# rvolden/C3POa

Measured on AMD Instinct MI355X. Metric: R2C2 reads->consensus/sec, higher is better.
Workload: dtype int32

## Files before the change

### c3poa_amd/csrc/c3_args.h

```cpp
#pragma once
#include "c3_dev.h"
#include <cstddef>

struct C3Counters {
  int queue;
  int peaks_queue;
  unsigned long long cells;
  unsigned long long cells_computed;
  unsigned long long zero_cells;
  int poa_ovf;
  int poa_ovf16;
  int n_windows;
  int win_ovf;
  int win_queue2;
  int band_layers, band_fallback;
  int band_mismatch;
  struct { int window, layer, R, q, band_row, full_row, next_row; } verify;
  unsigned long long phases[16];
};
static_assert(offsetof(C3Counters, cells) % 8 == 0 && offsetof(C3Counters, cells_computed) % 8 == 0 &&
              offsetof(C3Counters, zero_cells) % 8 == 0 && offsetof(C3Counters, phases) % 8 == 0, "u64 counters must be 8-byte aligned");

struct ConkArgs {
  C3Batch b; const uint8_t* sp_codes; const int* sp_len; int32_t* track; C3Info* info; C3Counters* cnt;
  int match, mismatch, penalty;
  int n_spl; int32_t* scan;
};
struct PeaksArgs {
  C3Batch b; const int32_t* track; C3Info* info; double* bufA; double* bufB; int32_t* cand; uint8_t* cstate;
  int32_t* raw_peaks; int32_t* n_raw; const int* sp_len; double coef[64]; int64_t maxL; int window, iters, min_dist;
  C3Counters* cnt;
};
struct PoaArgs {
  C3Batch b; C3Info* info; C3Params p; C3Counters* cnt; const int* work; int n_work;
  int* ibase; int* ebase; char* cellsb; uint8_t* bbase; long long* score;
  int Ncap, K, Pcap, cells_cap;
  uint8_t* draft; int32_t* tpos; uint8_t* msa_dbg; const int64_t* msa_off; int* msa_len;
  int rb_span;
  int no2col;
  uint4* desc; int* jump;
  int* pbase;
  int* overflow;
  int* overflow16;
};
#define C3_POA_NI 19
__host__ __device__ inline int c3_poa_far_shift(bool w32) { return w32 ? 0 : 2; }
struct PoaLayout { size_t ints, edges, cells, bases, score, desc, jump, path, total; };
__host__ __device__ inline PoaLayout c3_poa_layout(size_t Ncap, size_t K, int cells_cap, int far_shift, size_t Pcap) {
  PoaLayout l;
  l.ints = sizeof(int) * C3_POA_NI * Ncap; l.edges = sizeof(int) * 3 * Ncap * K;
  l.cells = 2 * (size_t)cells_cap + 16 * (size_t)(cells_cap >> far_shift);
  l.bases = 5 * Ncap; l.score = sizeof(long long) * Ncap; l.desc = sizeof(uint4) * 2 * Ncap;
  l.jump = sizeof(int) * C3_JUMP_LEVELS * Ncap; l.path = sizeof(int) * Pcap;
  l.total = l.ints + l.edges + l.cells + l.bases + l.score + l.desc + l.jump + l.path;
  return l;
}

struct WLayer { int qbeg, len, begin, end; };
struct WinRec { int rid, w, n_layers, blen, tgs, out_len, polished, pad_; };
struct PrepArgs {
  C3Batch b; C3Info* info; C3Params p; C3Counters* cnt; const int* work; int n_work;
  const uint8_t* draft; int32_t* tpos; int wcap; uint8_t* eD; int64_t ecap; int* lw_first; int* lw_last; int NLcap, NWcap;
  WinRec* wrec; WLayer* wlay; int* win_base;
  int sub_shift;
  int rows_old;
};
struct WinArgs {
  C3Batch b; C3Params p; C3Counters* cnt; int n_win; const WinRec* wrec_in; WinRec* wrec; const WLayer* wlay; int NLcap;
  const uint8_t* draft;
  uint8_t* base; int* ibase; int* ebase; long long* score;
  int32_t* H; uint16_t* D; uint4* rdesc; int Ncap, K; long long hcap; uint8_t* wout; int wout_cap;
  int Lcap;
  int band_mode;
  const int* wlist; int* ovf_list;
  int no_chain;
};
#define W_INTS 19
struct WinLayout { size_t ints, edges, bases, score, H, D, desc, total; };
__host__ __device__ inline WinLayout c3_win_layout(size_t Ncap, size_t K, size_t hcap) {
  WinLayout l;
  l.ints = sizeof(int) * W_INTS * Ncap; l.edges = sizeof(int) * 4 * Ncap * K; l.bases = 2 * Ncap; l.score = sizeof(long long) * Ncap;
  l.H = sizeof(int32_t) * hcap; l.D = hcap; l.desc = sizeof(uint4) * (Ncap + 1);
  l.total = l.ints + l.edges + l.bases + l.score + l.H + l.D + l.desc;
  return l;
}
struct StitchArgs {
  C3Batch b; C3Info* info; const int* work; int n_work; const WinRec* wrec; const int* win_base; const uint8_t* wout; int wout_cap; char* cons;
  const uint8_t* zflag;
};
struct AdapterArgs {
  C3Batch b; C3Params p; C3Counters* cnt;
  const uint8_t* ad_codes; const int* ad_len; int n_ad;
  uint8_t* D; long long dcap;
  int32_t* out;
};

struct ZeroArgs {
  C3Batch b; C3Info* info; C3Params p; C3Counters* cnt; const int* work; int n_work;
  uint8_t* D; long long dcap;
  int4* zinfo; uint8_t* zflag;
  const uint8_t* draft; char* cons;
  uint8_t* S; long long scap; int zk;
};

struct ZlLayout { long long ck, dir, car, total; };
__host__ __device__ inline ZlLayout c3_zl_layout(long long n0, long long n1, long long K) {
  ZlLayout l;
  l.ck = 0;
  l.dir = (n1 + K - 1) / K * (n0 + 1) * 8;
  l.car = (l.dir + (n1 < K ? n1 : K) * (n0 + 1) + 15) & ~15LL;
  l.total = (l.car + n1 * 12 + 255) & ~255LL;
  return l;
}
struct QvArgs {
  int n_reads; const C3Info* info; const uint32_t* pk; const int64_t* woff; const uint8_t* qual; const int64_t* off;
  const char* cons; char* qv;
  int sa_np, sa_n; const int64_t* sa_woff; const int64_t* sa_off; const int32_t* sa_mode;
  uint32_t* dirs; long long dir_words;
  int* gS; uint8_t* gcodes; long long gcap;
  int lds_n;
  unsigned long long* cnt;
};
```

### c3poa_amd/csrc/c3_stages.hip

```cpp
#include "c3_host.h"

__global__ void k_summary(const C3Info* info, const int64_t* off, int n, Summary* out) {
  int i = blockIdx.x * blockDim.x + threadIdx.x;
  if (i >= n) return;
  const C3Info* p = &info[i];
  Summary s; s.status = p->status; s.n_sub = p->n_sub; s.max_sub = 0; s.sum_sub = 0; s.max_dang = 0; s.n_peaks = p->n_peaks;
  for (int k = 0; k < p->n_sub; ++k) { int l = p->sub_end[k] - p->sub_beg[k]; s.sum_sub += l; if (l > s.max_sub) s.max_sub = l; }
  int L = (int)(off[i + 1] - off[i]);
  s.front = p->has_front ? p->front_end : 0; s.tail = p->has_tail ? L - p->tail_beg : 0;
  if (p->has_front) s.max_dang = p->front_end;
  if (p->has_tail && L - p->tail_beg > s.max_dang) s.max_dang = L - p->tail_beg;
  out[i] = s;
}

static hipError_t zero_counters(c3_handle* h) { return hipMemsetAsync(h->d_counter.p, 0, sizeof(C3Counters), h->stream); }

static int auto_slots(c3_handle* h, int want, size_t per_slot_bytes, int n_items, int waves_per_cu) {
  int s = want > 0 ? want : h->n_cus * waves_per_cu;
  size_t budget = h->mem_total ? h->mem_total / 3 : ((size_t)64 << 30);
  if (per_slot_bytes > 0) { size_t mx = budget / per_slot_bytes; if ((size_t)s > mx) s = (int)std::max<size_t>(mx, 1); }
  if (s > n_items) s = std::max(n_items, 1);
  return s;
}

static int run_conk(c3_handle* h) {
  HIPCHK(h->d_track.ensure(sizeof(int32_t) * (size_t)h->total + 64));
  HIPCHK(zero_cnt(h, &dev_cnt(h)->queue));
  ConkArgs a; a.b = dev_batch(h); a.sp_codes = h->d_sp_codes.as<uint8_t>(); a.sp_len = h->d_sp_len.as<int>();
  a.track = h->d_track.as<int32_t>(); a.info = h->d_info.as<C3Info>(); a.cnt = dev_cnt(h);
  a.match = h->cfg.conk_match; a.mismatch = h->cfg.conk_mismatch; a.penalty = h->cfg.conk_penalty; a.n_spl = h->n_spl; a.scan = nullptr;
  int waves = std::min(h->n, h->n_cus * 32);
  c3k_launch_conk(&a, h->max_spl, (waves + 3) / 4, 0, h->stream);
  HIPCHK(hipGetLastError());
  return 0;
}

static void savgol_coeffs(int window, double* c) {
  int m = (window - 1) / 2;
  double den = (double)(2 * m - 1) * (double)(2 * m + 1) * (double)(2 * m + 3);
  for (int k = -m; k <= 0; ++k) c[k + m] = 3.0 * (double)(3 * m * m + 3 * m - 1 - 5 * k * k) / den;
}

static int run_peaks(c3_handle* h) {
  static const int blocks_per_cu = c3k_peaks_blocks_per_cu();
  const int grid = std::min(h->n, h->n_cus * blocks_per_cu);
  h->peaks_grid = grid;
  const size_t mL = (size_t)h->maxL + 8;
  HIPCHK(h->d_bufA.ensure(sizeof(double) * mL * grid)); HIPCHK(h->d_bufB.ensure(sizeof(double) * mL * grid));
  HIPCHK(h->d_cand.ensure(sizeof(int32_t) * (mL / 2 + 2) * grid)); HIPCHK(h->d_cst.ensure((mL / 2 + 2) * grid));
  HIPCHK(h->d_raw.ensure(sizeof(int32_t) * (size_t)h->n * C3_MAX_PEAKS)); HIPCHK(h->d_nraw.ensure(sizeof(int32_t) * (size_t)h->n));
  PeaksArgs a; memset(&a, 0, sizeof(a));
  a.b = dev_batch(h); a.track = h->d_track.as<int32_t>(); a.info = h->d_info.as<C3Info>();
  a.bufA = h->d_bufA.as<double>(); a.bufB = h->d_bufB.as<double>(); a.cand = h->d_cand.as<int32_t>(); a.cstate = h->d_cst.as<uint8_t>();
  a.raw_peaks = h->d_raw.as<int32_t>(); a.n_raw = h->d_nraw.as<int32_t>(); a.sp_len = h->d_sp_len.as<int>();
  savgol_coeffs(h->cfg.sg_window, a.coef);
  a.maxL = (int64_t)mL; a.window = h->cfg.sg_window; a.iters = h->cfg.sg_iters; a.min_dist = h->cfg.mdistcutoff;
  a.cnt = dev_cnt(h);
  HIPCHK(zero_cnt(h, &a.cnt->peaks_queue));
  c3k_launch_peaks(&a, grid, h->stream);
  HIPCHK(hipGetLastError());
  return 0;
}

static int copy_summary(c3_handle* h) {
  const int n = h->n;
  HIPCHK(h->d_sum.ensure(sizeof(Summary) * (size_t)n));
  hipLaunchKernelGGL(k_summary, dim3((n + 255) / 256), dim3(256), 0, h->stream, h->d_info.as<C3Info>(), h->d_off.as<int64_t>(), n, h->d_sum.as<Summary>());
  h->sum.resize(n);
  HIPCHK(hipMemcpyAsync(h->sum.data(), h->d_sum.p, sizeof(Summary) * (size_t)n, hipMemcpyDeviceToHost, h->stream));
  if (!getenv("C3_NO_SPIN")) {
    hipError_t q;
    while ((q = hipStreamQuery(h->stream)) == hipErrorNotReady) { for (int k_ = 0; k_ < 64; ++k_) __builtin_ia32_pause(); }
    if (q != hipSuccess) HIPCHK(q);
  }
  HIPCHK(hipStreamSynchronize(h->stream));
  int k = 2;
  for (int i = 0; i < n; ++i) k = std::max(k, std::max(h->sum[i].n_peaks, h->sum[i].n_sub));
  h->res_prefix = std::min((k + 7) & ~7, (int)C3_MAX_PEAKS);
  return 0;
}

static void fill_zero_args(c3_handle* h, ZeroArgs& z, int nz) {
  memset(&z, 0, sizeof(z));
  z.b = dev_batch(h); z.info = h->d_info.as<C3Info>(); z.p = dev_params(h->cfg); z.cnt = dev_cnt(h);
  z.work = h->d_zwork.as<int>(); z.n_work = nz;
  z.D = h->s_zero_d.as<uint8_t>(); z.zinfo = h->d_zinfo.as<int4>(); z.zflag = h->d_zflag.as<uint8_t>();
  z.draft = h->d_draft.as<uint8_t>(); z.cons = h->d_cons.as<char>();
}

static const long long ZL_BUDGET = 1LL << 30;
static int run_zero(c3_handle* h) {
  h->zwork.clear();
  HIPCHK(h->d_zflag.ensure((size_t)h->n + 16));
  HIPCHK(hipMemsetAsync(h->d_zflag.p, 0, (size_t)h->n, h->stream));
  if (!h->cfg.zero || h->injected) return 0;
  const char* ev_long = getenv("C3_DEBUG_ZERO_LONG");
  const bool force_long = ev_long && atoi(ev_long) != 0;
  const char* ev_k = getenv("C3_DEBUG_ZERO_K");
  const int zk = (ev_k && atoi(ev_k) > 0) ? atoi(ev_k) : 256;
  long long dmax = 0, smax = 0;
  std::vector<int> zlong;
  for (int i = 0; i < h->n; ++i) {
    const Summary& s = h->sum[i];
    if (s.status != C3_ST_NO_CONSENSUS || s.n_sub != 0 || s.front <= 0 || s.tail <= 0) continue;
    const long long cells = (long long)s.front * s.tail;
    if (cells > h->cfg.zero_max_cells) continue;
    if (!force_long && s.front <= 4096 && cells <= (16 << 20)) {
      h->zwork.push_back(i);
      dmax = std::max(dmax, (long long)(s.front + 1) * (s.tail + 1));
    } else {
      zlong.push_back(i);
      smax = std::max(smax, c3_zl_layout(s.front, s.tail, zk).total);
    }
  }
  const int ns = (int)h->zwork.size(), nl = (int)zlong.size();
  h->zwork.insert(h->zwork.end(), zlong.begin(), zlong.end());
  const int nz = ns + nl;
  if (nz == 0) return 0;
  HIPCHK(h->d_zwork.ensure(sizeof(int) * (size_t)nz)); HIPCHK(h->d_zinfo.ensure(sizeof(int4) * (size_t)h->n));
  if (ns) {
    const int grid = std::min(ns, 512);
    HIPCHK(h->s_zero_d.ensure((size_t)dmax * grid + 64));
  }
  int grid_l = 0;
  if (nl) {
    grid_l = (int)std::min<long long>(std::min(nl, 2 * h->n_cus), std::max(1LL, ZL_BUDGET / smax));
    HIPCHK(h->s_zero_l.ensure((size_t)smax * grid_l));
  }
  HIPCHK(hipMemcpyAsync(h->d_zwork.p, h->zwork.data(), sizeof(int) * (size_t)nz, hipMemcpyHostToDevice, h->stream));
  if (ns) {
    ZeroArgs z; fill_zero_args(h, z, ns); z.dcap = dmax;
    DBG("zero: nz=%d grid=%d dmax=%lld\n", ns, std::min(ns, 512), dmax);
    c3k_launch_zero(&z, std::min(ns, 512), h->stream);
    HIPCHK(hipGetLastError());
  }
  if (nl) {
    ZeroArgs z; fill_zero_args(h, z, nl);
    z.work = h->d_zwork.as<int>() + ns; z.S = h->s_zero_l.as<uint8_t>(); z.scap = smax; z.zk = zk;
    DBG("zero long: nz=%d grid=%d slot=%lld K=%d\n", nl, grid_l, smax, zk);
    c3k_launch_zero_long(&z, grid_l, h->stream);
    HIPCHK(hipGetLastError());
  }
  { int r_ = copy_summary(h); DBG("zero done\n"); return r_; }
}

static int fetch_summary(c3_handle* h) {
  int rc = copy_summary(h);
  DBG("summary copied\n");
  if (rc) return rc;
  const auto wl0 = std::chrono::steady_clock::now();
  struct WlTimer { c3_handle* h; std::chrono::steady_clock::time_point t0; ~WlTimer() { h->tm.ms_host_worklist = std::chrono::duration<float, std::milli>(std::chrono::steady_clock::now() - t0).count(); } } wl_timer_{h, wl0};
  HIPCHK(zero_cnt(h, &dev_cnt(h)->zero_cells));
  if ((rc = run_zero(h))) return rc;
  const int n = h->n;
  h->work.clear();
  for (int i = 0; i < n; ++i) if (h->sum[i].status == C3_ST_OK && h->sum[i].n_sub >= 1) h->work.push_back(i);
  if (n < (1 << 24)) {
    const size_t m = h->work.size();
    std::vector<uint64_t> keys(m), tmp(m);
    for (size_t k = 0; k < m; ++k) {
      const int i = h->work[k];
      const uint64_t cost = (uint64_t)h->sum[i].sum_sub * (uint64_t)h->sum[i].n_sub;
      keys[k] = ((((uint64_t)1 << 40) - 1 - cost) << 24) | (uint64_t)i;
    }
    uint64_t* src = keys.data(); uint64_t* dst = tmp.data();
    for (int pass = 0; pass < 4; ++pass) {
      const int sh = 24 + 10 * pass;
      size_t cnt[1025] = {0};
      for (size_t k = 0; k < m; ++k) ++cnt[((src[k] >> sh) & 1023) + 1];
      for (int b = 0; b < 1024; ++b) cnt[b + 1] += cnt[b];
      for (size_t k = 0; k < m; ++k) dst[cnt[(src[k] >> sh) & 1023]++] = src[k];
      std::swap(src, dst);
    }
    for (size_t k = 0; k < m; ++k) h->work[k] = (int)(src[k] & 0xffffff);
  } else {
    std::stable_sort(h->work.begin(), h->work.end(), [&](int x, int y) {
      long cx = (long)h->sum[x].sum_sub * h->sum[x].n_sub, cy = (long)h->sum[y].sum_sub * h->sum[y].n_sub; return cx > cy; });
  }
  HIPCHK(h->d_work.ensure(sizeof(int) * std::max<size_t>(h->work.size(), 1)));
  if (!h->work.empty()) HIPCHK(hipMemcpyAsync(h->d_work.p, h->work.data(), sizeof(int) * h->work.size(), hipMemcpyHostToDevice, h->stream));
  return 0;
}

static int launch_poa(c3_handle* h, const int* d_work, int nw, int Ncap, int K, int Pcap, long long cells, int* d_overflow, int* d_overflow16, int waves_per_cu, int wide_ring) {
  cells = (cells + 15) & ~15LL;
  cells = (cells + 63) & ~63LL;
  const bool w32 = d_overflow16 == nullptr || getenv("C3_DEBUG_POA32");
  const PoaLayout L = c3_poa_layout(Ncap, K, (int)cells, c3_poa_far_shift(w32), Pcap);
  const int slots = auto_slots(h, h->cfg.slots_poa, L.total, nw, waves_per_cu);
  const size_t S = (size_t)slots;
  HIPCHK(h->s_poa_i.ensure(L.ints * S)); HIPCHK(h->s_poa_nk.ensure(L.edges * S));
  HIPCHK(h->s_poa_cells.ensure(L.cells * S + 256)); HIPCHK(h->s_poa_b.ensure(L.bases * S)); HIPCHK(h->s_poa_sc.ensure(L.score * S));
  HIPCHK(h->s_poa_desc.ensure(L.desc * S)); HIPCHK(h->s_poa_jump.ensure(L.jump * S)); HIPCHK(h->s_poa_path.ensure(L.path * S));
  PoaArgs a; memset(&a, 0, sizeof(a));
  a.b = dev_batch(h); a.info = h->d_info.as<C3Info>(); a.p = dev_params(h->cfg);
  a.cnt = dev_cnt(h); a.work = d_work; a.n_work = nw;
  a.ibase = h->s_poa_i.as<int>(); a.ebase = h->s_poa_nk.as<int>(); a.cellsb = h->s_poa_cells.as<char>();
  a.bbase = h->s_poa_b.as<uint8_t>(); a.score = h->s_poa_sc.as<long long>();
  a.Ncap = Ncap; a.K = K; a.Pcap = Pcap; a.cells_cap = (int)cells; a.desc = h->s_poa_desc.as<uint4>(); a.jump = h->s_poa_jump.as<int>();
  a.pbase = h->s_poa_path.as<int>(); a.overflow = d_overflow; a.overflow16 = d_overflow16;
  if (const char* e = getenv("C3_DEBUG_POA_RBSPAN")) a.rb_span = std::max(3300, atoi(e));
  a.no2col = getenv("C3_DEBUG_POA_NO2COL") != nullptr;
  a.draft = h->d_draft.as<uint8_t>(); a.tpos = h->d_tpos.as<int32_t>();
  a.msa_dbg = nullptr; a.msa_off = nullptr; a.msa_len = nullptr;
  if (h->debug_msa) { a.msa_dbg = h->d_msa.as<uint8_t>(); a.msa_off = h->d_msa_off.as<int64_t>(); a.msa_len = h->d_msa_len.as<int>(); }
  DBG("poa: nw=%d Ncap=%d K=%d cells=%lld slots=%d (%.1f MB per slot)%s\n", nw, Ncap, K, cells, slots, L.total / 1048576.0, d_overflow ? "" : (d_overflow16 ? " [full-size pass]" : " [32-bit pass]"));
  c3k_launch_poa(&a, slots, w32 ? 1 : 0, wide_ring, h->stream);
  HIPCHK(hipGetLastError());
  return 0;
}
// ... 268 lines not shown
```

### c3poa_amd/csrc/k_peaks.hip

```cpp
#include "c3_dev.h"
#include "c3_args.h"
#include "c3_launch.h"

#define PK_T 256
#define SG_T 1024
#define SG_H 64


__device__ __forceinline__ double sg_pad(const double* y, int n, int half, int x) {
  if (x < half) return y[0] - fabs(y[half - x] - y[0]);
  if (x >= n + half) return y[n - 1] + fabs(y[n - 2 - (x - n - half)] - y[n - 1]);
  return y[x - half];
}

__device__ __forceinline__ uint64_t dkey(double v) {
  uint64_t u = (uint64_t)__double_as_longlong(v);
  return (u >> 63) ? ~u : (u | 0x8000000000000000ull);
}
__device__ __forceinline__ double dunkey(uint64_t k) {
  uint64_t u = (k >> 63) ? (k & 0x7fffffffffffffffull) : ~k;
  return __longlong_as_double((long long)u);
}

__device__ __forceinline__ unsigned block_excl_scan(unsigned v, int* sh4, unsigned* total) {
  const int tid = threadIdx.x, lane = tid & 63, wv = tid >> 6;
  const unsigned inc = (unsigned)wave_scan_add((int)v);
  if (lane == 63) sh4[wv] = (int)inc;
  __syncthreads();
  unsigned base = 0, tot = 0;
#pragma unroll
  for (int w = 0; w < PK_T / 64; ++w) { const unsigned t = (unsigned)sh4[w]; if (w < wv) base += t; tot += t; }
  __syncthreads();
  *total = tot;
  return base + inc - v;
}

__device__ uint64_t block_select(const double* x, int n, int k, unsigned* hist, int* sh_i, uint64_t* keys ) {
  const int tid = threadIdx.x, lane = tid & 63;
  uint64_t prefix = 0, mask = 0;
  for (int pass = 7; pass >= 0; --pass) {
    const int shift = pass * 8;
    hist[tid] = 0;
    __syncthreads();
    for (int i0 = 0; i0 < n; i0 += 4 * PK_T) {
      double xv[4];
#pragma unroll
      for (int u = 0; u < 4; ++u) { const int i = i0 + u * PK_T + tid; xv[u] = i < n ? x[i] : 0.0; }
#pragma unroll
      for (int u = 0; u < 4; ++u) {
        const int i = i0 + u * PK_T + tid;
        const uint64_t key = dkey(xv[u]);
        const bool match = i < n && (key & mask) == prefix;
        const unsigned bin = (unsigned)(key >> shift) & 255u;
        unsigned long long todo = __ballot(match);
        for (int it = 0; it < 2 && todo; ++it) {
          const int l = __builtin_ctzll(todo);
          const unsigned b = (unsigned)__builtin_amdgcn_readlane((int)bin, l);
          const unsigned long long m = __ballot(match && bin == b) & todo;
          if (lane == l) atomicAdd(&hist[b], (unsigned)__popcll(m));
          todo &= ~m;
        }
        if (match && ((todo >> lane) & 1ull)) atomicAdd(&hist[bin], 1u);
      }
    }
    __syncthreads();
    {
      const unsigned c = hist[tid];
      unsigned tot;
      const unsigned cum = block_excl_scan(c, sh_i + 2, &tot);
      if (cum <= (unsigned)k && (unsigned)k < cum + c) { sh_i[0] = tid; sh_i[1] = (int)cum; sh_i[6] = (int)c; }
      if (tid == PK_T - 1 && (unsigned)k >= tot) { sh_i[0] = 255; sh_i[1] = (int)tot; sh_i[6] = INT32_MAX; }
    }
    __syncthreads();
    prefix |= (uint64_t)sh_i[0] << shift;
    mask |= (uint64_t)0xff << shift;
    k -= sh_i[1];
    const int cb = sh_i[6];
    __syncthreads();
    if (pass > 0 && cb <= PK_T) {
      if (tid == 0) sh_i[7] = 0;
      __syncthreads();
      for (int i0 = 0; i0 < n; i0 += 4 * PK_T) {
        double xv[4];
#pragma unroll
        for (int u = 0; u < 4; ++u) { const int i = i0 + u * PK_T + tid; xv[u] = i < n ? x[i] : 0.0; }
#pragma unroll
        for (int u = 0; u < 4; ++u) {
          const int i = i0 + u * PK_T + tid;
          const uint64_t key = dkey(xv[u]);
          if (i < n && (key & mask) == prefix) keys[atomicAdd(&sh_i[7], 1)] = key;
        }
      }
      __syncthreads();
      const uint64_t mine = tid < cb ? keys[tid] : ~0ull;
      int rank = 0;
      for (int j = 0; j < cb; ++j) { const uint64_t o = keys[j]; rank += (o < mine) || (o == mine && j < tid); }
      if (tid < cb && rank == k) *(uint64_t*)hist = mine;
      __syncthreads();
      const uint64_t r = *(const uint64_t*)hist;
      __syncthreads();
      return r;
    }
  }
  return prefix;
}

__device__ __forceinline__ int c3_rounding(int x, int base) {
  int q = x / base, r = x % base;
  if (2 * r < base) return q * base;
  if (2 * r > base) return (q + 1) * base;
  return ((q & 1) ? q + 1 : q) * base;
}

__global__ __launch_bounds__(PK_T) void k_peaks(PeaksArgs a) {
  __shared__ __attribute__((aligned(8))) unsigned hist[256];
  __shared__ int sh_i[8];
  __shared__ double sh_d[PK_T];
  __shared__ int sh_idx[PK_T];
  __shared__ int sh_cnt[PK_T + 1];
  __shared__ int kept[C3_MAX_PEAKS + 1];
  __shared__ double tb0[SG_T + 2 * SG_H], tb1[SG_T + 2 * SG_H];
  const int tid = threadIdx.x;
  double* A = a.bufA + (size_t)blockIdx.x * a.maxL;
  double* B = a.bufB + (size_t)blockIdx.x * a.maxL;
  int32_t* cand = a.cand + (size_t)blockIdx.x * (a.maxL / 2 + 2);
  uint8_t* cst = a.cstate + (size_t)blockIdx.x * (a.maxL / 2 + 2);
  const int half = (a.window - 1) / 2;

  __shared__ int s_rid;
  for (;;) {
    __syncthreads();
    if (tid == 0) s_rid = atomicAdd(&a.cnt->peaks_queue, 1);
    __syncthreads();
    const int rid = s_rid;
    if (rid >= a.b.n) break;
    C3Info* info = &a.info[rid];
    if (info->status == C3_ST_NOT_ASSIGNED) { if (tid == 0) a.n_raw[rid] = 0; continue; }
    const int64_t off = a.b.off[rid];
    const int n = (int)(a.b.off[rid + 1] - off);
    if (n < half + 1 || n < 2) { if (tid == 0) { info->status = C3_ST_TOO_SHORT; a.n_raw[rid] = 0; } continue; }
    const int32_t* tr = a.track + off;
    double* src = A; double* dst = B;
    const int H = a.iters * half;
    if (a.iters >= 1 && H <= SG_H) {
      double* xout = (a.iters & 1) ? B : A;
      for (int t0 = 0; t0 < n; t0 += SG_T) {
        const int base = t0 - H;
        const int T = min(SG_T, n - t0);
        for (int x = tid; x < T + 2 * H; x += PK_T) { const int g = base + x; if (g >= 0 && g < n) tb0[x] = (double)tr[g]; }
        __syncthreads();
        double* sb = tb0; double* db = tb1;
        for (int it = 0; it < a.iters; ++it) {
          const int ext = (a.iters - 1 - it) * half;
          const int glo = max(0, t0 - ext), ghi = min(n, t0 + T + ext);
          const bool last = it == a.iters - 1;
          const double* yv = sb - base;
          for (int g = glo + tid; g < ghi; g += PK_T) {
            double acc = 0.0;
            if (g >= half && g + half < n) {
              const double* y = yv + (g - half);
              if (half == 20) {
#pragma unroll
                for (int k = 0; k < 20; ++k) acc = __builtin_fma(a.coef[k], y[k] + y[40 - k], acc);
                acc = __builtin_fma(a.coef[20], y[20], acc);
              } else {
                for (int k = 0; k < half; ++k) acc = __builtin_fma(a.coef[k], y[k] + y[2 * half - k], acc);
                acc = __builtin_fma(a.coef[half], y[half], acc);
              }
            } else {
              for (int k = 0; k < half; ++k)
                acc = __builtin_fma(a.coef[k], sg_pad(yv, n, half, g + k) + sg_pad(yv, n, half, g + 2 * half - k), acc);
              acc = __builtin_fma(a.coef[half], sg_pad(yv, n, half, g + half), acc);
            }
            if (last) xout[g] = acc; else db[g - base] = acc;
          }
          __syncthreads();
          double* t = sb; sb = db; db = t;
        }
      }
      src = xout;
      __syncthreads();
    } else {
    for (int i = tid; i < n; i += PK_T) A[i] = (double)tr[i];
    __syncthreads();
    for (int it = 0; it < a.iters; ++it) {
      for (int i = tid; i < n; i += PK_T) {
        double acc = 0.0;
        if (i >= half && i + half < n) {
          const double* y = src + (i - half);
          for (int k = 0; k < half; ++k) acc = __builtin_fma(a.coef[k], y[k] + y[2 * half - k], acc);
          acc = __builtin_fma(a.coef[half], y[half], acc);
        } else {
          for (int k = 0; k < half; ++k)
            acc = __builtin_fma(a.coef[k], sg_pad(src, n, half, i + k) + sg_pad(src, n, half, i + 2 * half - k), acc);
          acc = __builtin_fma(a.coef[half], sg_pad(src, n, half, i + half), acc);
        }
        dst[i] = acc;
      }
      __syncthreads();
      double* t = src; src = dst; dst = t;
    }
    }
    const double* x = src;
    double med;
    {
#ifdef C3_EXP_X2_SEL
      { volatile uint64_t sink_ = block_select(x, n, (n - 1) / 3, hist, sh_i, (uint64_t*)sh_d); (void)sink_; }
#endif
      uint64_t k1 = block_select(x, n, (n - 1) / 2, hist, sh_i, (uint64_t*)sh_d);
      double v1 = dunkey(k1);
      if (n & 1) med = v1;
      else {
        int cnt_le = 0; uint64_t mn = ~0ull;
        for (int i = tid; i < n; i += PK_T) {
          uint64_t key = dkey(x[i]);
          if (key <= k1) ++cnt_le; else if (key < mn) mn = key;
        }
        sh_cnt[tid] = cnt_le; sh_d[tid] = __longlong_as_double((long long)mn);
        __syncthreads();
        for (int s = PK_T / 2; s > 0; s >>= 1) {
          if (tid < s) {
            sh_cnt[tid] += sh_cnt[tid + s];
            uint64_t o = (uint64_t)__double_as_longlong(sh_d[tid + s]), m = (uint64_t)__double_as_longlong(sh_d[tid]);
            if (o < m) sh_d[tid] = sh_d[tid + s];
          }
          __syncthreads();
        }
        int tot_le = sh_cnt[0]; uint64_t mnk = (uint64_t)__double_as_longlong(sh_d[0]);
        __syncthreads();
        double v2 = (tot_le > n / 2) ? v1 : dunkey(mnk);
        med = (v1 + v2) / 2.0;
      }
    }
    double mx = -1.0e308;
    for (int i = tid; i < n; i += PK_T) mx = fmax(mx, x[i]);
    sh_d[tid] = mx;
    __syncthreads();
    for (int s = PK_T / 2; s > 0; s >>= 1) { if (tid < s) sh_d[tid] = fmax(sh_d[tid], sh_d[tid + s]); __syncthreads(); }
    mx = sh_d[0];
    __syncthreads();
    int n_kept = 0;
    if (!(mx < 6 * med)) {
      const double height = med * 3;
      const int chunk = (n + PK_T - 1) / PK_T;
      const int lo = max(1, tid * chunk), hi = min(n - 1, (tid + 1) * chunk);
      int cnt = 0;
      for (int pass = 0; pass < 2; ++pass) {
        int w = (pass == 1) ? sh_cnt[tid] : 0;
        for (int i = lo; i < hi; ++i) {
          if (x[i - 1] < x[i]) {
            int ia = i + 1;
            while (ia < n - 1 && x[ia] == x[i]) ++ia;
            if (x[ia] < x[i] && x[i] >= height) {
              if (pass == 0) ++cnt; else { cand[w] = (i + ia - 1) / 2; cst[w] = 1; ++w; }
            }
          }
        }
        if (pass == 0) {
          unsigned tot;
          const unsigned ex = block_excl_scan((unsigned)cnt, sh_i + 2, &tot);
          sh_cnt[tid] = (int)ex;
          if (tid == 0) sh_cnt[PK_T] = (int)tot;
          __syncthreads();
        }
      }
      const int nc = sh_cnt[PK_T];
      __syncthreads();
      const int dist = a.min_dist < 1 ? 1 : a.min_dist;
      for (;;) {
        double bv = -1.0e308; int bi = -1;
        for (int c = tid; c < nc; c += PK_T)
          if (cst[c] == 1) { double v = x[cand[c]]; if (v > bv || (v == bv && c > bi)) { bv = v; bi = c; } }
        sh_d[tid] = bv; sh_idx[tid] = bi;
        __syncthreads();
        for (int s = PK_T / 2; s > 0; s >>= 1) {
          if (tid < s) {
            double ov = sh_d[tid + s]; int oi = sh_idx[tid + s];
            if (oi >= 0 && (sh_idx[tid] < 0 || ov > sh_d[tid] || (ov == sh_d[tid] && oi > sh_idx[tid]))) { sh_d[tid] = ov; sh_idx[tid] = oi; }
          }
          __syncthreads();
        }
        const int win = sh_idx[0];
        __syncthreads();
        if (win < 0) break;
        const int wp = cand[win];
        if (tid == 0) { cst[win] = 2; if (n_kept < C3_MAX_PEAKS) kept[n_kept] = wp; }
        ++n_kept;
        for (int c = tid; c < nc; c += PK_T)
          if (cst[c] == 1) { int dlt = cand[c] - wp; if (dlt < 0) dlt = -dlt; if (dlt < dist) cst[c] = 0; }
        __syncthreads();
      }
    }
    if (tid == 0) {
      int status = C3_ST_OK;
      if (n_kept > C3_MAX_PEAKS - 1) { status = C3_ST_LIMIT; n_kept = 0; }
      for (int i = 1; i < n_kept; ++i) { int v = kept[i], k = i - 1; while (k >= 0 && kept[k] > v) { kept[k + 1] = kept[k]; --k; } kept[k + 1] = v; }
      a.n_raw[rid] = n_kept;
      for (int i = 0; i < n_kept; ++i) a.raw_peaks[(size_t)rid * C3_MAX_PEAKS + i] = kept[i];
      const int S = a.sp_len[a.b.splint_id[rid]];
      int np = 0;
      for (int i = 0; i < n_kept; ++i) { int p = kept[i] + S / 2; if (p < n) info->peaks[np++] = p; }
      info->n_peaks = np;
      int ns = 0, hf = 0, ht = 0, fe = 0, tb = 0;
      if (status == C3_ST_OK && np == 0) status = C3_ST_NO_PEAKS;
      if (np > 1) {
        const int nl = np - 1;
        int* r = sh_idx;
        int* srt = sh_cnt;
        for (int i = 0; i < nl; ++i) srt[i] = r[i] = c3_rounding(info->peaks[i + 1] - info->peaks[i], 50);
        for (int i = 1; i < nl; ++i) { int v = srt[i], k = i - 1; while (k >= 0 && srt[k] > v) { srt[k + 1] = srt[k]; --k; } srt[k + 1] = v; }
        const double med2 = (nl & 1) ? (double)srt[nl / 2] : ((double)srt[nl / 2 - 1] + (double)srt[nl / 2]) / 2.0;
        const double lo8 = med2 * 0.8, hi12 = med2 * 1.2;
        for (int i = 0; i < nl; ++i)
          if (lo8 <= (double)r[i] && (double)r[i] <= hi12) { info->sub_beg[ns] = info->peaks[i]; info->sub_end[ns] = info->peaks[i + 1]; ++ns; }
        if (info->peaks[0] > 100) { hf = 1; fe = info->peaks[0]; }
        if (n - info->peaks[np - 1] > 100) { ht = 1; tb = info->peaks[np - 1]; }
      } else if (np == 1) {
        hf = 1; fe = info->peaks[0]; ht = 1; tb = info->peaks[0];
      }
      info->n_sub = ns; info->has_front = hf; info->has_tail = ht; info->front_end = fe; info->tail_beg = tb;
      if (status == C3_ST_OK && ns == 0) status = C3_ST_NO_CONSENSUS;
      if (status == C3_ST_OK && ns > C3_MAX_SUB) status = C3_ST_LIMIT;
      info->status = status;
    }
    __syncthreads();
  }
}

extern "C" int c3k_peaks_blocks_per_cu(void) {
  int nb = 0;
  if (hipOccupancyMaxActiveBlocksPerMultiprocessor(&nb, k_peaks, PK_T, 0) != hipSuccess || nb < 1) { (void)hipGetLastError(); nb = 4; }
  return nb;
}
extern "C" void c3k_launch_peaks(const PeaksArgs* a, int grid, hipStream_t stream) {
  hipLaunchKernelGGL(k_peaks, dim3(grid), dim3(PK_T), 0, stream, *a);
}
```

Before: 426,800.

## Use sample-bucket median and LDS candidate peak picking in peaks kernel

Replaces the eight-pass radix selection for the median with a sample-based bucket histogram that gathers only the median's bucket into shared memory, falling back to radix select when the bucket overflows. The max is now folded into the final FIR pass. Peak candidates are collected into shared memory and picked by a single wave, with no global cand/cstate passes or block-wide reductions, and the old path is kept as an overflow fallback. It also sets waves_per_eu, reuses the FIR tiles as scratch, and uses a per-read buffer row when the grid covers every read. This adds code complexity and fallback branches, and the changed shared-memory aliasing and tie-breaking could alter results.

```diff
diff --git a/c3poa_amd/csrc/c3_args.h b/c3poa_amd/csrc/c3_args.h
--- a/c3poa_amd/csrc/c3_args.h
+++ b/c3poa_amd/csrc/c3_args.h
@@ -30,7 +30,12 @@
   C3Batch b; const int32_t* track; C3Info* info; double* bufA; double* bufB; int32_t* cand; uint8_t* cstate;
   int32_t* raw_peaks; int32_t* n_raw; const int* sp_len; double coef[64]; int64_t maxL; int window, iters, min_dist;
   C3Counters* cnt;
+  int kcap;
+  int ccap;
+  int old_path;
 };
+#define C3_PEAKS_KCAP 1152
+#define C3_PEAKS_CCAP 1024
 struct PoaArgs {
   C3Batch b; C3Info* info; C3Params p; C3Counters* cnt; const int* work; int n_work;
   int* ibase; int* ebase; char* cellsb; uint8_t* bbase; long long* score;
diff --git a/c3poa_amd/csrc/c3_stages.hip b/c3poa_amd/csrc/c3_stages.hip
--- a/c3poa_amd/csrc/c3_stages.hip
+++ b/c3poa_amd/csrc/c3_stages.hip
@@ -43,7 +43,8 @@
 
 static int run_peaks(c3_handle* h) {
   static const int blocks_per_cu = c3k_peaks_blocks_per_cu();
-  const int grid = std::min(h->n, h->n_cus * blocks_per_cu);
+  int grid = std::min(h->n, h->n_cus * blocks_per_cu);
+  if (const char* g = getenv("C3_DEBUG_PEAKS_GRID")) grid = std::max(1, std::min(grid, atoi(g)));
   h->peaks_grid = grid;
   const size_t mL = (size_t)h->maxL + 8;
   HIPCHK(h->d_bufA.ensure(sizeof(double) * mL * grid)); HIPCHK(h->d_bufB.ensure(sizeof(double) * mL * grid));
@@ -56,6 +57,10 @@
   savgol_coeffs(h->cfg.sg_window, a.coef);
   a.maxL = (int64_t)mL; a.window = h->cfg.sg_window; a.iters = h->cfg.sg_iters; a.min_dist = h->cfg.mdistcutoff;
   a.cnt = dev_cnt(h);
+  const char* dbg = getenv("C3_DEBUG_PEAKS"); const char* kc = getenv("C3_DEBUG_PEAKS_KCAP"); const char* cc = getenv("C3_DEBUG_PEAKS_CCAP");
+  a.old_path = dbg && !strcmp(dbg, "old");
+  a.kcap = kc ? std::min(std::max(atoi(kc), 1), C3_PEAKS_KCAP) : C3_PEAKS_KCAP;
+  a.ccap = cc ? std::min(std::max(atoi(cc), 1), C3_PEAKS_CCAP) : C3_PEAKS_CCAP;
   HIPCHK(zero_cnt(h, &a.cnt->peaks_queue));
   c3k_launch_peaks(&a, grid, h->stream);
   HIPCHK(hipGetLastError());
diff --git a/c3poa_amd/csrc/k_peaks.hip b/c3poa_amd/csrc/k_peaks.hip
--- a/c3poa_amd/csrc/k_peaks.hip
+++ b/c3poa_amd/csrc/k_peaks.hip
@@ -5,6 +5,11 @@
 #define PK_T 256
 #define SG_T 1024
 #define SG_H 64
+#define PK_TB (SG_T + 2 * SG_H)
+#define PK_NB 1024
+static_assert(PK_NB == 4 * PK_T && PK_NB * sizeof(unsigned) <= PK_TB * sizeof(double), "one thread scans four buckets; histogram inside tile 0");
+static_assert(C3_PEAKS_KCAP <= PK_TB, "the gathered bucket aliases the second FIR tile");
+static_assert(C3_PEAKS_CCAP <= PK_TB && C3_PEAKS_CCAP * sizeof(int) <= PK_TB * sizeof(double), "candidate values alias tile 0, positions tile 1");
 
 
 __device__ __forceinline__ double sg_pad(const double* y, int n, int half, int x) {
@@ -22,8 +27,8 @@
   return __longlong_as_double((long long)u);
 }
 
-__device__ __forceinline__ unsigned block_excl_scan(unsigned v, int* sh4, unsigned* total) {
-  const int tid = threadIdx.x, lane = tid & 63, wv = tid >> 6;
+__device__ __forceinline__ unsigned block_excl_scan(int tid, unsigned v, int* sh4, unsigned* total) {
+  const int lane = tid & 63, wv = tid >> 6;
   const unsigned inc = (unsigned)wave_scan_add((int)v);
   if (lane == 63) sh4[wv] = (int)inc;
   __syncthreads();
@@ -35,8 +40,27 @@
   return base + inc - v;
 }
 
-__device__ uint64_t block_select(const double* x, int n, int k, unsigned* hist, int* sh_i, uint64_t* keys ) {
-  const int tid = threadIdx.x, lane = tid & 63;
+__device__ __forceinline__ void hist_add(int tid, unsigned* hist, bool match, unsigned bin) {
+  const int lane = tid & 63;
+  unsigned long long todo = __ballot(match);
+  for (int it = 0; it < 2 && todo; ++it) {
+    const int l = __builtin_ctzll(todo);
+    const unsigned b = (unsigned)__builtin_amdgcn_readlane((int)bin, l);
+    const unsigned long long m = __ballot(match && bin == b) & todo;
+    if (lane == l) atomicAdd(&hist[b], (unsigned)__popcll(m));
+    todo &= ~m;
+  }
+  if (match && ((todo >> lane) & 1ull)) atomicAdd(&hist[bin], 1u);
+}
+
+__device__ __forceinline__ void rank_two(int tid, const uint64_t mine, const uint64_t* keys, int cb, int ka, int kb, uint64_t* res) {
+  int rank = 0;
+  for (int j = 0; j < cb; ++j) { const uint64_t o = keys[j]; rank += (o < mine) || (o == mine && j < tid); }
+  if (tid < cb && rank == ka) res[0] = mine;
+  if (tid < cb && rank == kb) res[1] = mine;
+}
+
+__device__ uint64_t block_select(int tid, const double* x, int n, int k, unsigned* hist, int* sh_i, uint64_t* keys ) {
   uint64_t prefix = 0, mask = 0;
   for (int pass = 7; pass >= 0; --pass) {
     const int shift = pass * 8;
@@ -50,24 +74,14 @@
       for (int u = 0; u < 4; ++u) {
         const int i = i0 + u * PK_T + tid;
         const uint64_t key = dkey(xv[u]);
-        const bool match = i < n && (key & mask) == prefix;
-        const unsigned bin = (unsigned)(key >> shift) & 255u;
-        unsigned long long todo = __ballot(match);
-        for (int it = 0; it < 2 && todo; ++it) {
-          const int l = __builtin_ctzll(todo);
-          const unsigned b = (unsigned)__builtin_amdgcn_readlane((int)bin, l);
-          const unsigned long long m = __ballot(match && bin == b) & todo;
-          if (lane == l) atomicAdd(&hist[b], (unsigned)__popcll(m));
-          todo &= ~m;
-        }
-        if (match && ((todo >> lane) & 1ull)) atomicAdd(&hist[bin], 1u);
+        hist_add(tid, hist, i < n && (key & mask) == prefix, (unsigned)(key >> shift) & 255u);
       }
     }
     __syncthreads();
     {
       const unsigned c = hist[tid];
       unsigned tot;
-      const unsigned cum = block_excl_scan(c, sh_i + 2, &tot);
+      const unsigned cum = block_excl_scan(tid, c, sh_i + 2, &tot);
       if (cum <= (unsigned)k && (unsigned)k < cum + c) { sh_i[0] = tid; sh_i[1] = (int)cum; sh_i[6] = (int)c; }
       if (tid == PK_T - 1 && (unsigned)k >= tot) { sh_i[0] = 255; sh_i[1] = (int)tot; sh_i[6] = INT32_MAX; }
     }
@@ -92,10 +106,7 @@
         }
       }
       __syncthreads();
-      const uint64_t mine = tid < cb ? keys[tid] : ~0ull;
-      int rank = 0;
-      for (int j = 0; j < cb; ++j) { const uint64_t o = keys[j]; rank += (o < mine) || (o == mine && j < tid); }
-      if (tid < cb && rank == k) *(uint64_t*)hist = mine;
+      rank_two(tid, tid < cb ? keys[tid] : ~0ull, keys, cb, k, k + 1, (uint64_t*)hist);
       __syncthreads();
       const uint64_t r = *(const uint64_t*)hist;
       __syncthreads();
@@ -103,6 +114,137 @@
     }
   }
   return prefix;
+}
+
+__device__ double median_radix(int tid, const double* x, int n, unsigned* hist, int* sh_i, double* sh_d, int* sh_cnt) {
+#ifdef C3_EXP_X2_SEL
+  { volatile uint64_t sink_ = block_select(tid, x, n, (n - 1) / 3, hist, sh_i, (uint64_t*)sh_d); (void)sink_; }
+#endif
+  const uint64_t k1 = block_select(tid, x, n, (n - 1) / 2, hist, sh_i, (uint64_t*)sh_d);
+  const double v1 = dunkey(k1);
+  if (n & 1) return v1;
+  int cnt_le = 0; uint64_t mn = ~0ull;
+  for (int i = tid; i < n; i += PK_T) {
+    uint64_t key = dkey(x[i]);
+    if (key <= k1) ++cnt_le; else if (key < mn) mn = key;
+  }
+  sh_cnt[tid] = cnt_le; sh_d[tid] = __longlong_as_double((long long)mn);
+  __syncthreads();
+  for (int s = PK_T / 2; s > 0; s >>= 1) {
+    if (tid < s) {
+      sh_cnt[tid] += sh_cnt[tid + s];
+      uint64_t o = (uint64_t)__double_as_longlong(sh_d[tid + s]), m = (uint64_t)__double_as_longlong(sh_d[tid]);
+      if (o < m) sh_d[tid] = sh_d[tid + s];
+    }
+    __syncthreads();
+  }
+  const int tot_le = sh_cnt[0]; const uint64_t mnk = (uint64_t)__double_as_longlong(sh_d[0]);
+  __syncthreads();
+  const double v2 = (tot_le > n / 2) ? v1 : dunkey(mnk);
+  return (v1 + v2) / 2.0;
+}
+
+__device__ bool median_buckets(int tid, const double* x, int n, int kcap, double* med,
+                               unsigned* bh , double* vals , unsigned* hist, int* sh_i, double* sh_d) {
+  const int lane = tid & 63, wv = tid >> 6;
+  const int k = (n - 1) / 2;
+  const bool even = !(n & 1);
+  uint64_t* res = (uint64_t*)hist;
+  int B = 0, kk = k, cb = n;
+  double lo = 0.0, s = 0.0;
+#define PK_BUCKET(v) ({ const double t_ = ((v) - lo) * s; t_ >= (double)(PK_NB - 1) ? PK_NB - 1 : max((int)t_, 0); })
+  if (n > PK_T) {
+    uint64_t* skeys = (uint64_t*)sh_d;
+    const uint64_t mine = dkey(x[(int)(((long long)tid * n) >> 8)]);
+    skeys[tid] = mine;
+    __syncthreads();
+    rank_two(tid, mine, skeys, PK_T, PK_T / 4, 3 * PK_T / 4 - 1, res);
+    __syncthreads();
+    lo = dunkey(res[0]);
+    const double hi = dunkey(res[1]);
+    if (!(hi > lo)) { __syncthreads(); return false; }
+    s = (double)PK_NB / (hi - lo);
+    if (!(s < 1.0e300)) { __syncthreads(); return false; }
+#pragma unroll
+    for (int u = 0; u < 4; ++u) bh[u * PK_T + tid] = 0;
+    __syncthreads();
+    for (int i0 = 0; i0 < n; i0 += 4 * PK_T) {
+      double xv[4];
+#pragma unroll
+      for (int u = 0; u < 4; ++u) { const int i = i0 + u * PK_T + tid; xv[u] = i < n ? x[i] : lo; }
+#pragma unroll
+      for (int u = 0; u < 4; ++u) {
+        const bool in = i0 + u * PK_T + tid < n;
+        const int b = PK_BUCKET(xv[u]);
+        const unsigned long long m0 = __ballot(in && b == 0), m1 = __ballot(in && b == PK_NB - 1);
+        if (lane == 0 && m0) atomicAdd(&bh[0], (unsigned)__popcll(m0));
+        if (lane == 0 && m1) atomicAdd(&bh[PK_NB - 1], (unsigned)__popcll(m1));
+        if (in && b != 0 && b != PK_NB - 1) atomicAdd(&bh[b], 1u);
+      }
+    }
+    __syncthreads();
+    {
+      unsigned c[4], sum = 0, tot;
+#pragma unroll
+      for (int u = 0; u < 4; ++u) { c[u] = bh[4 * tid + u]; sum += c[u]; }
+      unsigned cum = block_excl_scan(tid, sum, sh_i + 2, &tot);
+#pragma unroll
+      for (int u = 0; u < 4; ++u) {
+        if (cum <= (unsigned)k && (unsigned)k < cum + c[u]) { sh_i[0] = 4 * tid + u; sh_i[1] = (int)cum; sh_i[6] = (int)c[u]; }
+        cum += c[u];
+      }
+    }
+    __syncthreads();
+    B = sh_i[0]; kk = k - sh_i[1]; cb = sh_i[6];
+  }
+  if (cb > kcap) { __syncthreads(); return false; }
+  __syncthreads();
+  if (tid == 0) sh_i[7] = 0;
+  __syncthreads();
+  uint64_t above = ~0ull;
+  for (int i0 = 0; i0 < n; i0 += 4 * PK_T) {
+    double xv[4];
+#pragma unroll
+    for (int u = 0; u < 4; ++u) { const int i = i0 + u * PK_T + tid; xv[u] = i < n ? x[i] : lo; }
+#pragma unroll
+    for (int u = 0; u < 4; ++u) {
+      const int i = i0 + u * PK_T + tid;
+      const int b = n > PK_T ? PK_BUCKET(xv[u]) : 0;
+      if (i < n && b == B) { const int slot = atomicAdd(&sh_i[7], 1); if (slot < kcap) vals[slot] = xv[u]; }
+      if (i < n && b > B) { const uint64_t key = dkey(xv[u]); if (key < above) above = key; }
+    }
+  }
+#undef PK_BUCKET
+  __syncthreads();
+  const bool second_inside = kk + 1 < cb;
+  uint64_t k1, k2 = 0;
+  if (cb <= PK_T) {
+    uint64_t* keys = (uint64_t*)vals;
+    const uint64_t mine = tid < cb ? dkey(vals[tid]) : ~0ull;
+    if (tid < cb) keys[tid] = mine;
+    __syncthreads();
+    rank_two(tid, mine, keys, cb, kk, kk + 1, res);
+    __syncthreads();
+    k1 = res[0]; k2 = res[1];
+  } else {
+    k1 = block_select(tid, vals, cb, kk, hist, sh_i, (uint64_t*)sh_d);
+    if (even && second_inside) k2 = block_select(tid, vals, cb, kk + 1, hist, sh_i, (uint64_t*)sh_d);
+  }
+  if (even && !second_inside) {
+    uint64_t* ex = (uint64_t*)sh_d;
+#pragma unroll
+    for (int o = 32; o > 0; o >>= 1) { const uint64_t t = (uint64_t)__shfl_xor((unsigned long long)above, o); if (t < above) above = t; }
+    __syncthreads();
+    if (lane == 0) ex[wv] = above;
+    __syncthreads();
+    k2 = ex[0];
+#pragma unroll
+    for (int w = 1; w < PK_T / 64; ++w) if (ex[w] < k2) k2 = ex[w];
+  }
+  __syncthreads();
+  const double v1 = dunkey(k1);
+  *med = even ? (v1 + dunkey(k2)) / 2.0 : v1;
+  return true;
 }
 
 __device__ __forceinline__ int c3_rounding(int x, int base) {
@@ -112,38 +254,50 @@
   return ((q & 1) ? q + 1 : q) * base;
 }
 
-__global__ __launch_bounds__(PK_T) void k_peaks(PeaksArgs a) {
+__global__ __launch_bounds__(PK_T) __attribute__((amdgpu_waves_per_eu(6, 6))) void k_peaks(PeaksArgs a) {
   __shared__ __attribute__((aligned(8))) unsigned hist[256];
   __shared__ int sh_i[8];
   __shared__ double sh_d[PK_T];
   __shared__ int sh_idx[PK_T];
   __shared__ int sh_cnt[PK_T + 1];
   __shared__ int kept[C3_MAX_PEAKS + 1];
-  __shared__ double tb0[SG_T + 2 * SG_H], tb1[SG_T + 2 * SG_H];
-  const int tid = threadIdx.x;
-  double* A = a.bufA + (size_t)blockIdx.x * a.maxL;
-  double* B = a.bufB + (size_t)blockIdx.x * a.maxL;
+  __shared__ double tb[2 * PK_TB];
+  __shared__ int s_hdr[2];
+  double* const tb0 = tb; double* const tb1 = tb + PK_TB;
   int32_t* cand = a.cand + (size_t)blockIdx.x * (a.maxL / 2 + 2);
   uint8_t* cst = a.cstate + (size_t)blockIdx.x * (a.maxL / 2 + 2);
   const int half = (a.window - 1) / 2;
-
-  __shared__ int s_rid;
+  const bool rows_by_read = a.b.n <= (int)gridDim.x;
+
   for (;;) {
-    __syncthreads();
-    if (tid == 0) s_rid = atomicAdd(&a.cnt->peaks_queue, 1);
-    __syncthreads();
-    const int rid = s_rid;
+    int tid = threadIdx.x;
+    asm volatile("" : "+v"(tid));
+    const int lane = tid & 63, wv = tid >> 6;
+    __syncthreads();
+    if (tid == 0) {
+      const int r = atomicAdd(&a.cnt->peaks_queue, 1);
+      s_hdr[0] = r; s_hdr[1] = r < a.b.n ? a.info[r].status : 0;
+    }
+    __syncthreads();
+    const int rid = s_hdr[0];
     if (rid >= a.b.n) break;
     C3Info* info = &a.info[rid];
-    if (info->status == C3_ST_NOT_ASSIGNED) { if (tid == 0) a.n_raw[rid] = 0; continue; }
+    if (s_hdr[1] == C3_ST_NOT_ASSIGNED) { if (tid == 0) a.n_raw[rid] = 0; continue; }
     const int64_t off = a.b.off[rid];
     const int n = (int)(a.b.off[rid + 1] - off);
     if (n < half + 1 || n < 2) { if (tid == 0) { info->status = C3_ST_TOO_SHORT; a.n_raw[rid] = 0; } continue; }
     const int32_t* tr = a.track + off;
+    double* A = a.bufA + (size_t)(rows_by_read ? rid : (int)blockIdx.x) * a.maxL;
+    double* B = a.bufB + (size_t)(rows_by_read ? rid : (int)blockIdx.x) * a.maxL;
     double* src = A; double* dst = B;
+    double mx = -1.0e308;
     const int H = a.iters * half;
-    if (a.iters >= 1 && H <= SG_H) {
+    const bool tiled = a.iters >= 1 && H <= SG_H;
+    if (tiled) {
       double* xout = (a.iters & 1) ? B : A;
+#ifdef C3_EXP_X2_FIR
+      for (int rep_ = 0; rep_ < 2; ++rep_)
+#endif
       for (int t0 = 0; t0 < n; t0 += SG_T) {
         const int base = t0 - H;
         const int T = min(SG_T, n - t0);
@@ -172,7 +326,7 @@
                 acc = __builtin_fma(a.coef[k], sg_pad(yv, n, half, g + k) + sg_pad(yv, n, half, g + 2 * half - k), acc);
               acc = __builtin_fma(a.coef[half], sg_pad(yv, n, half, g + half), acc);
             }
-            if (last) xout[g] = acc; else db[g - base] = acc;
+            if (last) { xout[g] = acc; mx = fmax(mx, acc); } else db[g - base] = acc;
           }
           __syncthreads();
           double* t = sb; sb = db; db = t;
@@ -202,46 +356,92 @@
     }
     }
     const double* x = src;
-    double med;
-    {
-#ifdef C3_EXP_X2_SEL
-      { volatile uint64_t sink_ = block_select(x, n, (n - 1) / 3, hist, sh_i, (uint64_t*)sh_d); (void)sink_; }
+    double med = 0.0;
+    bool radix = a.old_path;
+    if (!radix) {
+      if (!tiled) for (int i = tid; i < n; i += PK_T) mx = fmax(mx, x[i]);
+#pragma unroll
+      for (int o = 32; o > 0; o >>= 1) mx = fmax(mx, __shfl_xor(mx, o));
+      if (lane == 0) sh_d[wv] = mx;
+      __syncthreads();
+      mx = fmax(fmax(sh_d[0], sh_d[1]), fmax(sh_d[2], sh_d[3]));
+      __syncthreads();
+#ifdef C3_EXP_X2_MED
+      { double m_; (void)median_buckets(tid, x, n, a.kcap, &m_, (unsigned*)tb0, tb1, hist, sh_i, sh_d); }
 #endif
-      uint64_t k1 = block_select(x, n, (n - 1) / 2, hist, sh_i, (uint64_t*)sh_d);
-      double v1 = dunkey(k1);
-      if (n & 1) med = v1;
-      else {
-        int cnt_le = 0; uint64_t mn = ~0ull;
-        for (int i = tid; i < n; i += PK_T) {
-          uint64_t key = dkey(x[i]);
-          if (key <= k1) ++cnt_le; else if (key < mn) mn = key;
-        }
-        sh_cnt[tid] = cnt_le; sh_d[tid] = __longlong_as_double((long long)mn);
-        __syncthreads();
-        for (int s = PK_T / 2; s > 0; s >>= 1) {
-          if (tid < s) {
-            sh_cnt[tid] += sh_cnt[tid + s];
-            uint64_t o = (uint64_t)__double_as_longlong(sh_d[tid + s]), m = (uint64_t)__double_as_longlong(sh_d[tid]);
-            if (o < m) sh_d[tid] = sh_d[tid + s];
-          }
-          __syncthreads();
-        }
-        int tot_le = sh_cnt[0]; uint64_t mnk = (uint64_t)__double_as_longlong(sh_d[0]);
-        __syncthreads();
-        double v2 = (tot_le > n / 2) ? v1 : dunkey(mnk);
-        med = (v1 + v2) / 2.0;
-      }
-    }
-    double mx = -1.0e308;
-    for (int i = tid; i < n; i += PK_T) mx = fmax(mx, x[i]);
-    sh_d[tid] = mx;
-    __syncthreads();
-    for (int s = PK_T / 2; s > 0; s >>= 1) { if (tid < s) sh_d[tid] = fmax(sh_d[tid], sh_d[tid + s]); __syncthreads(); }
-    mx = sh_d[0];
-    __syncthreads();
+      radix = !median_buckets(tid, x, n, a.kcap, &med, (unsigned*)tb0, tb1, hist, sh_i, sh_d);
+    }
+    if (radix) med = median_radix(tid, x, n, hist, sh_i, sh_d, sh_cnt);
+    if (a.old_path) {
+      mx = -1.0e308;
+      for (int i = tid; i < n; i += PK_T) mx = fmax(mx, x[i]);
+      sh_d[tid] = mx;
+      __syncthreads();
+      for (int s = PK_T / 2; s > 0; s >>= 1) { if (tid < s) sh_d[tid] = fmax(sh_d[tid], sh_d[tid + s]); __syncthreads(); }
+      mx = sh_d[0];
+      __syncthreads();
+    }
     int n_kept = 0;
     if (!(mx < 6 * med)) {
       const double height = med * 3;
+      const int dist = a.min_dist < 1 ? 1 : a.min_dist;
+      double* cval = tb0; int* cpos = (int*)tb1;
+      int nc = a.ccap + 1;
+      if (!a.old_path)
+#ifdef C3_EXP_X2_CAND
+      for (int rep_ = 0; rep_ < 2; ++rep_)
+#endif
+      {
+        if (tid == 0) sh_i[7] = 0;
+        __syncthreads();
+        for (int i0 = 1; i0 < n - 1; i0 += 4 * PK_T) {
+          double xl[4], xc[4];
+#pragma unroll
+          for (int u = 0; u < 4; ++u) {
+            const int i = i0 + u * PK_T + tid;
+            const bool in = i < n - 1;
+            xl[u] = in ? x[i - 1] : 0.0; xc[u] = in ? x[i] : 0.0;
+          }
+#pragma unroll
+          for (int u = 0; u < 4; ++u) {
+            const int i = i0 + u * PK_T + tid;
+            if (i < n - 1 && xl[u] < xc[u] && xc[u] >= height) {
+              int ia = i + 1;
+              while (ia < n - 1 && x[ia] == xc[u]) ++ia;
+              if (x[ia] < xc[u]) {
+                const int slot = atomicAdd(&sh_i[7], 1);
+                if (slot < a.ccap) { cval[slot] = xc[u]; cpos[slot] = (i + ia - 1) / 2; }
+              }
+            }
+          }
+        }
+        __syncthreads();
+        nc = sh_i[7];
+        __syncthreads();
+      }
+      if (nc <= a.ccap) {
+        if (wv == 0) {
+          for (;;) {
+            double bv = -HUGE_VAL; int bp = -1;
+            for (int c = lane; c < nc; c += 64) {
+              const int p = cpos[c];
+              if (p >= 0) { const double v = cval[c]; if (bp < 0 || v > bv || (v == bv && p > bp)) { bv = v; bp = p; } }
+            }
+            double wvmax = bv;
+#pragma unroll
+            for (int o = 32; o > 0; o >>= 1) wvmax = fmax(wvmax, __shfl_xor(wvmax, o));
+            const int wp = wave_max((bp >= 0 && bv == wvmax) ? bp : -1);
+            if (wp < 0) break;
+            if (lane == 0 && n_kept < C3_MAX_PEAKS) kept[n_kept] = wp;
+            ++n_kept;
+            for (int c = lane; c < nc; c += 64) {
+              const int p = cpos[c];
+              if (p >= 0) { int dlt = p - wp; if (dlt < 0) dlt = -dlt; if (dlt < dist) cpos[c] = -1; }
+            }
+          }
+        }
+        __syncthreads();
+      } else {
       const int chunk = (n + PK_T - 1) / PK_T;
       const int lo = max(1, tid * chunk), hi = min(n - 1, (tid + 1) * chunk);
       int cnt = 0;
@@ -258,18 +458,17 @@
         }
         if (pass == 0) {
           unsigned tot;
-          const unsigned ex = block_excl_scan((unsigned)cnt, sh_i + 2, &tot);
+          const unsigned ex = block_excl_scan(tid, (unsigned)cnt, sh_i + 2, &tot);
           sh_cnt[tid] = (int)ex;
           if (tid == 0) sh_cnt[PK_T] = (int)tot;
           __syncthreads();
         }
       }
-      const int nc = sh_cnt[PK_T];
-      __syncthreads();
-      const int dist = a.min_dist < 1 ? 1 : a.min_dist;
+      const int ncg = sh_cnt[PK_T];
+      __syncthreads();
       for (;;) {
         double bv = -1.0e308; int bi = -1;
-        for (int c = tid; c < nc; c += PK_T)
+        for (int c = tid; c < ncg; c += PK_T)
           if (cst[c] == 1) { double v = x[cand[c]]; if (v > bv || (v == bv && c > bi)) { bv = v; bi = c; } }
         sh_d[tid] = bv; sh_idx[tid] = bi;
         __syncthreads();
@@ -286,9 +485,10 @@
         const int wp = cand[win];
         if (tid == 0) { cst[win] = 2; if (n_kept < C3_MAX_PEAKS) kept[n_kept] = wp; }
         ++n_kept;
-        for (int c = tid; c < nc; c += PK_T)
+        for (int c = tid; c < ncg; c += PK_T)
           if (cst[c] == 1) { int dlt = cand[c] - wp; if (dlt < 0) dlt = -dlt; if (dlt < dist) cst[c] = 0; }
         __syncthreads();
+      }
       }
     }
     if (tid == 0) {
@@ -298,27 +498,28 @@
       a.n_raw[rid] = n_kept;
       for (int i = 0; i < n_kept; ++i) a.raw_peaks[(size_t)rid * C3_MAX_PEAKS + i] = kept[i];
       const int S = a.sp_len[a.b.splint_id[rid]];
+      int* pk = (int*)hist;
       int np = 0;
-      for (int i = 0; i < n_kept; ++i) { int p = kept[i] + S / 2; if (p < n) info->peaks[np++] = p; }
+      for (int i = 0; i < n_kept; ++i) { int p = kept[i] + S / 2; if (p < n) { pk[np] = p; info->peaks[np] = p; ++np; } }
       info->n_peaks = np;
-      int ns = 0, hf = 0, ht = 0, fe = 0, tb = 0;
+      int ns = 0, hf = 0, ht = 0, fe = 0, tb_ = 0;
       if (status == C3_ST_OK && np == 0) status = C3_ST_NO_PEAKS;
       if (np > 1) {
         const int nl = np - 1;
         int* r = sh_idx;
         int* srt = sh_cnt;
-        for (int i = 0; i < nl; ++i) srt[i] = r[i] = c3_rounding(info->peaks[i + 1] - info->peaks[i], 50);
+        for (int i = 0; i < nl; ++i) srt[i] = r[i] = c3_rounding(pk[i + 1] - pk[i], 50);
         for (int i = 1; i < nl; ++i) { int v = srt[i], k = i - 1; while (k >= 0 && srt[k] > v) { srt[k + 1] = srt[k]; --k; } srt[k + 1] = v; }
         const double med2 = (nl & 1) ? (double)srt[nl / 2] : ((double)srt[nl / 2 - 1] + (double)srt[nl / 2]) / 2.0;
         const double lo8 = med2 * 0.8, hi12 = med2 * 1.2;
         for (int i = 0; i < nl; ++i)
-          if (lo8 <= (double)r[i] && (double)r[i] <= hi12) { info->sub_beg[ns] = info->peaks[i]; info->sub_end[ns] = info->peaks[i + 1]; ++ns; }
-        if (info->peaks[0] > 100) { hf = 1; fe = info->peaks[0]; }
-        if (n - info->peaks[np - 1] > 100) { ht = 1; tb = info->peaks[np - 1]; }
+          if (lo8 <= (double)r[i] && (double)r[i] <= hi12) { info->sub_beg[ns] = pk[i]; info->sub_end[ns] = pk[i + 1]; ++ns; }
+        if (pk[0] > 100) { hf = 1; fe = pk[0]; }
+        if (n - pk[np - 1] > 100) { ht = 1; tb_ = pk[np - 1]; }
       } else if (np == 1) {
-        hf = 1; fe = info->peaks[0]; ht = 1; tb = info->peaks[0];
-      }
-      info->n_sub = ns; info->has_front = hf; info->has_tail = ht; info->front_end = fe; info->tail_beg = tb;
+        hf = 1; fe = pk[0]; ht = 1; tb_ = pk[0];
+      }
+      info->n_sub = ns; info->has_front = hf; info->has_tail = ht; info->front_end = fe; info->tail_beg = tb_;
       if (status == C3_ST_OK && ns == 0) status = C3_ST_NO_CONSENSUS;
       if (status == C3_ST_OK && ns > C3_MAX_SUB) status = C3_ST_LIMIT;
       info->status = status;
```

Result: no change. 428,700 (median of 4 runs) (+0.4%).
